# TIERS/multi-modal-loam

Hardware: AMD Instinct MI355X
Metric: scans/s (feature-extract+kNN+10 GN iters) on 16-ring x1800 + Livox 24k fused cloud (higher is better)
Workload: dtype f32/f64; 1 GPU; BASELINE configs[1]: fused VLP-16 16x1800 + Livox Horizon 24000 scan (52800 pts), local map 200000 pts, 1 association pass (thres_dist 25), 10 GN iterations, W=1; resident_slots=8192, stream_lanes=2, distinct_scans=64, map_tiles_touched=43, map_tiles_complete=43, parallelism=scan-sharded x1, device=AMD Radeon Graphics, cus=256

## Files before the change

multi-modal-loam_amd/csrc/knn5_dev.h:

```cpp

__device__ __forceinline__ int cell_coord(float v, float o, float inv, int dim) {
    int c = (int)floorf((v - o) * inv);
    return c < 0 ? 0 : (c >= dim ? dim - 1 : c);
}

struct Knn5 {
    unsigned long long key[5];
};
constexpr unsigned long long KNN_EMPTY = (0x7f800000ull << 32) | 0x7fffffffull;
__device__ __forceinline__ unsigned long long knn_key(float d, int id) {
    return ((unsigned long long)__float_as_uint(d) << 32) | (unsigned)id;
}
__device__ __forceinline__ float knn_d(const Knn5& k, int j) { return __uint_as_float((unsigned)(k.key[j] >> 32)); }
__device__ __forceinline__ int knn_id(const Knn5& k, int j) { return (int)(unsigned)k.key[j]; }
__device__ __forceinline__ void knn_init(Knn5& k) {
#pragma unroll
    for (int i = 0; i < 5; ++i) k.key[i] = KNN_EMPTY;
}
__device__ __forceinline__ unsigned long long sel64(bool c, unsigned long long a, unsigned long long b) {
    const unsigned lo = __builtin_unpredictable(c) ? (unsigned)a : (unsigned)b;
    const unsigned hi = __builtin_unpredictable(c) ? (unsigned)(a >> 32) : (unsigned)(b >> 32);
    return ((unsigned long long)hi << 32) | lo;
}
__device__ __forceinline__ void knn_insert_key(Knn5& k, unsigned long long x) {
    const bool lt0 = x < k.key[0], lt1 = x < k.key[1], lt2 = x < k.key[2], lt3 = x < k.key[3], lt4 = x < k.key[4];
    const unsigned long long c1 = sel64(lt0, k.key[0], x), c2 = sel64(lt1, k.key[1], x), c3 = sel64(lt2, k.key[2], x),
                             c4 = sel64(lt3, k.key[3], x);
    k.key[4] = sel64(lt4, c4, k.key[4]);
    k.key[3] = sel64(lt3, c3, k.key[3]);
    k.key[2] = sel64(lt2, c2, k.key[2]);
    k.key[1] = sel64(lt1, c1, k.key[1]);
    k.key[0] = sel64(lt0, x, k.key[0]);
}
__device__ __forceinline__ void knn_insert(Knn5& k, float dd, int ii) {
    const unsigned long long x = knn_key(dd, ii);
    if (!(x < k.key[4])) return;
    knn_insert_key(k, x);
}

__device__ __forceinline__ void scan_range(const float4* __restrict__ pts, const uint16_t* __restrict__ tags, int mytag,
                                           int s, int e, float qx, float qy, float qz, Knn5& k) {
    for (int i0 = s; i0 < e; i0 += 4) {
        float4 p[4];
        int tg[4];
#pragma unroll
        for (int u = 0; u < 4; ++u) {
            const unsigned i = (unsigned)min(i0 + u, e - 1);
            p[u] = pts[i];
            tg[u] = tags ? (int)tags[i] : mytag;
        }
#pragma unroll
        for (int u = 0; u < 4; ++u) {
            float dx = qx - p[u].x, dy = qy - p[u].y, dz = qz - p[u].z;
            float r = 0;
            r += dx * dx;
            r += dy * dy;
            r += dz * dz;
            const unsigned long long x = (i0 + u >= e || tg[u] != mytag) ? ~0ull : knn_key(r, (int)__float_as_uint(p[u].w));
            if (x < k.key[4]) knn_insert_key(k, x);
        }
    }
}

struct KnnQuery {
    float qx, qy, qz, inset;
    float fx, fy, fz;
    int hx, hy, hz;
};

__device__ __forceinline__ KnnQuery knn_query(const MmlGrid& g, float qx, float qy, float qz) {
    KnnQuery q;
    q.qx = qx;
    q.qy = qy;
    q.qz = qz;
    const float fx = (qx - g.origin[0]) * g.inv_cell, fy = (qy - g.origin[1]) * g.inv_cell,
                fz = (qz - g.origin[2]) * g.inv_cell;
    q.fx = fx;
    q.fy = fy;
    q.fz = fz;
    q.hx = (int)floorf(fx);
    q.hy = (int)floorf(fy);
    q.hz = (int)floorf(fz);
    float inset = fminf(fminf(fminf(fx - q.hx, q.hx + 1 - fx), fminf(fy - q.hy, q.hy + 1 - fy)),
                        fminf(fz - q.hz, q.hz + 1 - fz));
    q.inset = (inset > 0.f) ? inset : 0.f;
    return q;
}

__device__ __forceinline__ bool knn_done(const MmlGrid& g, float inset, int r, float d5, float max_d2) {
    float rho = ((float)r + inset) * g.cell;
    rho = rho - 1e-3f * g.cell;
    if (!(rho > 0.f)) return false;
    const float rho2 = rho * rho;
    return d5 < rho2 || rho2 >= max_d2;
}

__device__ __forceinline__ void scan_shell_row(const MmlGrid& g, const KnnQuery& q, int r, int y, int z, Knn5& k,
                                               int mytag = -1, float bound = INFINITY) {
    const int DX = g.dim[0], DY = g.dim[1], DZ = g.dim[2];
    if (y < 0 || y >= DY || z < 0 || z >= DZ) return;
    int xlo = -1, xhi = DX;
    if (bound < INFINITY) {
        const float gy = y > q.hy ? (float)y - q.fy : (y < q.hy ? q.fy - (float)(y + 1) : 0.f);
        const float gz = z > q.hz ? (float)z - q.fz : (z < q.hz ? q.fz - (float)(z + 1) : 0.f);
        const float reach = sqrtf(bound * 1.00001f) * g.inv_cell + 4e-3f;
        const float w2 = reach * reach - (gy * gy + gz * gz);
        if (w2 < 0.f) return;
        const float w = sqrtf(w2);
        xlo = (int)floorf(fmaxf(q.fx - w, -1.f));
        xhi = (int)floorf(fminf(q.fx + w, (float)DX));
    }
    const int x0 = q.hx - r, x1 = q.hx + r;
    const bool face = (z == q.hz - r || z == q.hz + r || y == q.hy - r || y == q.hy + r);
    const int rowbase = DX * (y + DY * z);
    if (face) {
        const int xa = max(max(x0, 0), xlo), xb = min(min(x1, DX - 1), xhi);
        if (xa <= xb)
            scan_range(g.pts, g.tags, mytag, g.cell_start[rowbase + xa], g.cell_start[rowbase + xb + 1], q.qx, q.qy, q.qz, k);
    } else {
        if (x0 >= 0 && x0 < DX && x0 >= xlo)
            scan_range(g.pts, g.tags, mytag, g.cell_start[rowbase + x0], g.cell_start[rowbase + x0 + 1], q.qx, q.qy, q.qz, k);
        if (x1 >= 0 && x1 < DX && x1 != x0 && x1 <= xhi)
            scan_range(g.pts, g.tags, mytag, g.cell_start[rowbase + x1], g.cell_start[rowbase + x1 + 1], q.qx, q.qy, q.qz, k);
    }
}

template <int STRIDE>
__device__ __forceinline__ void scan_shell_rows4(const MmlGrid& g, const KnnQuery& q, int r, int ylo, int wy, int zlo, int nrows,
                                                 int t, Knn5& k, int mytag, float bound) {
    const int DX = g.dim[0], DY = g.dim[1];
    const float reach = sqrtf(bound * 1.00001f) * g.inv_cell + 4e-3f;
    const float reach2 = reach * reach;
    const int x0 = q.hx - r, x1 = q.hx + r;
    unsigned ia[8], ib[8];
#pragma unroll
    for (int u = 0; u < 4; ++u) {
        const int tu = t + u * STRIDE;
        const int y = ylo + tu % wy, z = zlo + tu / wy;
        const float gy = y > q.hy ? (float)y - q.fy : (y < q.hy ? q.fy - (float)(y + 1) : 0.f);
        const float gz = z > q.hz ? (float)z - q.fz : (z < q.hz ? q.fz - (float)(z + 1) : 0.f);
        const float w2 = reach2 - (gy * gy + gz * gz);
        const bool in = tu < nrows && !(w2 < 0.f);
        const float w = sqrtf(fmaxf(w2, 0.f));
        const int xlo = (int)floorf(fmaxf(q.fx - w, -1.f)), xhi = (int)floorf(fminf(q.fx + w, (float)DX));
        const bool face = (z == q.hz - r || z == q.hz + r || y == q.hy - r || y == q.hy + r);
        const int rowbase = DX * (y + DY * z);
        const int xa = max(max(x0, 0), xlo), xb = min(min(x1, DX - 1), xhi);
        const bool va = in && (face ? xa <= xb : (x0 >= 0 && x0 < DX && x0 >= xlo));
        const bool vb = in && !face && x1 >= 0 && x1 < DX && x1 != x0 && x1 <= xhi;
        ia[2 * u] = va ? (unsigned)(rowbase + (face ? xa : x0)) : 0u;
        ib[2 * u] = va ? (unsigned)(rowbase + (face ? xb : x0) + 1) : 0u;
        ia[2 * u + 1] = vb ? (unsigned)(rowbase + x1) : 0u;
        ib[2 * u + 1] = vb ? (unsigned)(rowbase + x1 + 1) : 0u;
    }
    int s[8], e[8];
#pragma unroll
    for (int v = 0; v < 8; ++v) {
        s[v] = g.cell_start[ia[v]];
        e[v] = g.cell_start[ib[v]];
    }
    unsigned todo = 0;
#pragma unroll
    for (int v = 0; v < 8; ++v) todo |= (s[v] < e[v] ? 1u : 0u) << v;
#pragma unroll 1
    while (todo) {
        const int v = __ffs((int)todo) - 1;
        todo &= todo - 1;
        int ss = s[0], ee = e[0];
#pragma unroll
        for (int j = 1; j < 8; ++j) {
            ss = v == j ? s[j] : ss;
            ee = v == j ? e[j] : ee;
        }
        scan_range(g.pts, g.tags, mytag, ss, ee, q.qx, q.qy, q.qz, k);
    }
}

__device__ __constant__ const signed char kRing1Row[9][2] = {{0, 0}, {-1, 0}, {1, 0}, {0, -1}, {0, 1}, {-1, -1}, {1, -1}, {-1, 1}, {1, 1}};

__device__ __forceinline__ bool scan_rings01(const MmlGrid& g, const KnnQuery& q, int rmax, float max_d2, Knn5& k, int mytag) {
    scan_shell_row(g, q, 0, q.hy, q.hz, k, mytag);
    if (knn_done(g, q.inset, 0, knn_d(k, 4), max_d2)) return true;
    if (rmax < 1) return false;
#pragma unroll 1
    for (int t = 0; t < 9; ++t) scan_shell_row(g, q, 1, q.hy + kRing1Row[t][0], q.hz + kRing1Row[t][1], k, mytag, knn_d(k, 4));
    return knn_done(g, q.inset, 1, knn_d(k, 4), max_d2);
}

__device__ __forceinline__ unsigned long long knn_head(const Knn5& k, int head) {
    unsigned long long key = KNN_EMPTY;
#pragma unroll
    for (int s = 0; s < 5; ++s)
        if (head == s) key = k.key[s];
    return key;
}
__device__ __forceinline__ unsigned long long shfl_xor_u64(unsigned long long v, int o) {
    const unsigned lo = __shfl_xor((unsigned)v, o), hi = __shfl_xor((unsigned)(v >> 32), o);
    return ((unsigned long long)hi << 32) | lo;
}
template <int SPAN>
__device__ __forceinline__ void lanes_merge5(const Knn5& local, Knn5& out) {
    int head = 0;
#pragma unroll
    for (int r = 0; r < 5; ++r) {
        const unsigned long long mine = knn_head(local, head);
        unsigned long long m = mine;
#pragma unroll
        for (int o = SPAN / 2; o > 0; o >>= 1) {
            const unsigned long long other = shfl_xor_u64(m, o);
            m = other < m ? other : m;
        }
        out.key[r] = m;
        if (mine == m && (unsigned)(m >> 32) < 0x7f800000u) head++;
    }
}

__device__ void knn5_search(const MmlGrid& g, bool valid, float qx, float qy, float qz, float max_d2, Knn5& k) {
    knn_init(k);
    const KnnQuery q = knn_query(g, qx, qy, qz);
    const int rgrid = max(max(max(q.hx, g.dim[0] - 1 - q.hx), max(q.hy, g.dim[1] - 1 - q.hy)), max(q.hz, g.dim[2] - 1 - q.hz));
    const float rf = ceilf(sqrtf(max_d2) * g.inv_cell) + 1.f;
    const int rmax = rf < (float)rgrid ? (int)rf : max(rgrid, 0);
    bool pending = false;
    if (valid) {
        pending = !scan_rings01(g, q, rmax, max_d2, k, -1);
        if (rmax < 2) pending = false;
    }
    unsigned long long todo = __ballot(pending);
    const int lane = threadIdx.x & 63;
    while (todo) {
        const int src = __ffsll((long long)todo) - 1;
        todo &= todo - 1;
        KnnQuery s;
        s.qx = __shfl(q.qx, src);
        s.qy = __shfl(q.qy, src);
        s.qz = __shfl(q.qz, src);
        s.inset = __shfl(q.inset, src);
        s.fx = __shfl(q.fx, src);
        s.fy = __shfl(q.fy, src);
        s.fz = __shfl(q.fz, src);
        s.hx = __shfl(q.hx, src);
        s.hy = __shfl(q.hy, src);
        s.hz = __shfl(q.hz, src);
        Knn5 loc;
        if (lane == src)
            loc = k;
        else
            knn_init(loc);
        Knn5 best;
        knn_init(best);
        const int rmax_s = __shfl(rmax, src);
        const int rnear = max(max(max(-s.hx, s.hx - (g.dim[0] - 1)), max(-s.hy, s.hy - (g.dim[1] - 1))),
                              max(-s.hz, s.hz - (g.dim[2] - 1)));
        for (int r = max(2, rnear); r <= rmax_s; ++r) {
            const float bnd = fminf(knn_d(best, 4), __shfl(knn_d(k, 4), src));
            const int ylo = max(s.hy - r, 0), yhi = min(s.hy + r, g.dim[1] - 1), zlo = max(s.hz - r, 0), zhi = min(s.hz + r, g.dim[2] - 1);
            const int wy = yhi - ylo + 1, wz = zhi - zlo + 1;
            if (wy > 0 && wz > 0)
                for (int t = lane; t < wy * wz; t += 64)
                    scan_shell_row(g, s, r, ylo + (t % wy), zlo + (t / wy), loc, -1, fminf(bnd, knn_d(loc, 4)));
            lanes_merge5<64>(loc, best);
            if (knn_done(g, s.inset, r, knn_d(best, 4), max_d2)) break;
        }
        if (lane == src) k = best;
    }
}
```

multi-modal-loam_amd/csrc/map_assoc.hip:

```cpp
#include <math.h>
#include <stdlib.h>

#include <cstring>
#include <string.h>

#include "mml_internal.h"
#include "voxel_sort_dev.h"

namespace {

struct GridDev {
    float ox, oy, oz, inv_cell, cell;
    int dx, dy, dz, ncell;
};

#include "knn5_dev.h"

__global__ void k_cell_keys(const float4* pts, int m, GridDev g, unsigned* keys, unsigned* vals) {
    int i = blockIdx.x * blockDim.x + threadIdx.x;
    if (i >= m) return;
    float4 p = pts[i];
    int cx = cell_coord(p.x, g.ox, g.inv_cell, g.dx);
    int cy = cell_coord(p.y, g.oy, g.inv_cell, g.dy);
    int cz = cell_coord(p.z, g.oz, g.inv_cell, g.dz);
// ... 324 lines not shown
    float a11 = 0, a12 = 0, a13 = 0, a22 = 0, a23 = 0, a33 = 0;
#pragma unroll
    for (int j = 0; j < 5; j++) {
        float ax = nx[j] - cx, ay = ny[j] - cy, az = nz[j] - cz;
        a11 += ax * ax;
        a12 += ax * ay;
        a13 += ax * az;
        a22 += ay * ay;
        a23 += ay * az;
        a33 += az * az;
    }
    a11 /= 5;
    a12 /= 5;
    a13 /= 5;
    a22 /= 5;
    a23 /= 5;
    a33 /= 5;
    double ud[3];
    eig3_sym(a11, a12, a22, a13, a23, a33, m.ev, ud);
    m.cx = cx;
    m.cy = cy;
    m.cz = cz;
    if (!(m.ev[2] > 3 * m.ev[1])) return false;
    m.p1[0] = cx + 0.1 * ud[0];
    m.p1[1] = cy + 0.1 * ud[1];
    m.p1[2] = cz + 0.1 * ud[2];
    m.p2[0] = cx - 0.1 * ud[0];
    m.p2[1] = cy - 0.1 * ud[1];
    m.p2[2] = cz - 0.1 * ud[2];
    return true;
}

struct PlaneModel5 {
    double X[3];
    float pa, pb, pc, pd;
    double proj[3];
};
__device__ __forceinline__ bool plane_model5(const float* nx, const float* ny, const float* nz, float sx, float sy, float sz,
                                             PlaneModel5& m) {
    double A[5][3];
#pragma unroll
    for (int j = 0; j < 5; j++) {
        A[j][0] = nx[j];
        A[j][1] = ny[j];
        A[j][2] = nz[j];
    }
    plane_fit5(A, m.X);
    float pa = m.X[0], pb = m.X[1], pc = m.X[2], pd = 1;
    float ps = sqrtf(pa * pa + pb * pb + pc * pc);
    pa /= ps;
    pb /= ps;
    pc /= ps;
    pd /= ps;
    m.pa = pa;
    m.pb = pb;
    m.pc = pc;
    m.pd = pd;
    bool planeValid = true;
#pragma unroll
    for (int j = 0; j < 5; j++) {
        if (fabs((double)(pa * nx[j] + pb * ny[j] + pc * nz[j] + pd)) > 0.2) {
            planeValid = false;
            break;
        }
    }
    if (!planeValid) return false;
    double dist = pa * sx + pb * sy + pc * sz + pd;
    m.proj[0] = (double)sx - dist * (double)pa;
    m.proj[1] = (double)sy - dist * (double)pb;
    m.proj[2] = (double)sz - dist * (double)pc;
    return true;
}

__device__ __forceinline__ bool fit_and_store(const AssocParams& P, int kind, int b, int i, const float4 f, const double* T,
                                              float sx, float sy, float sz, bool ok, const Knn5& k, const float4* mp) {
    if (kind == 0) {
        MmlLineFactor out;
        out.src = -1;
        out.error = 0;
        if (ok) {
            float nx[5], ny[5], nz[5];
#pragma unroll
            for (int j = 0; j < 5; j++) {
                float4 q = mp[knn_id(k, j)];
                nx[j] = q.x;
                ny[j] = q.y;
                nz[j] = q.z;
            }
            LineModel5 m;
            if (line_model5(nx, ny, nz, m)) {
                const float x1 = m.p1[0], y1 = m.p1[1], z1 = m.p1[2], x2 = m.p2[0], y2 = m.p2[1], z2 = m.p2[2];
                out.ori[0] = f.x;
                out.ori[1] = f.y;
                out.ori[2] = f.z;
                out.p1[0] = x1;
                out.p1[1] = y1;
                out.p1[2] = z1;
                out.p2[0] = x2;
                out.p2[1] = y2;
                out.p2[2] = z2;
                out.src = i;
                double Px, Py, Pz;
                tf_point(T, f.x, f.y, f.z, Px, Py, Pz);
                double ax = x1, ay = y1, az = z1, bx = x2, by = y2, bz = z2;
                double l12 = sqrt((ax - bx) * (ax - bx) + (ay - by) * (ay - by) + (az - bz) * (az - bz));
                double c0 = (Px - ax) * (Py - by) - (Px - bx) * (Py - ay);
                double c1 = (Px - ax) * (Pz - bz) - (Px - bx) * (Pz - az);
                double c2 = (Py - ay) * (Pz - bz) - (Py - by) * (Pz - az);
                double a012 = sqrt(c0 * c0 + c1 * c1 + c2 * c2);
                out.error = a012 / l12;
            }
        }
        if (out.src >= 0) P.lf[(size_t)b * P.MF + i] = out;
        return out.src >= 0;
    } else {
        MmlPlaneFactor out;
        out.src = -1;
        out.error = 0;
        out._pad = 0;
        if (ok) {
            float nx[5], ny[5], nz[5];
#pragma unroll
            for (int j = 0; j < 5; j++) {
                float4 q = mp[knn_id(k, j)];
                nx[j] = q.x;
                ny[j] = q.y;
                nz[j] = q.z;
            }
            PlaneModel5 m;
            if (plane_model5(nx, ny, nz, sx, sy, sz, m)) {
                out.ori[0] = f.x;
                out.ori[1] = f.y;
                out.ori[2] = f.z;
                out.omega[0] = m.pa;
                out.omega[1] = m.pb;
                out.omega[2] = m.pc;
                out.proj[0] = m.proj[0];
                out.proj[1] = m.proj[1];
                out.proj[2] = m.proj[2];
                double Px, Py, Pz;
                tf_point(T, f.x, f.y, f.z, Px, Py, Pz);
                double ex = Px - out.proj[0], ey = Py - out.proj[1], ez = Pz - out.proj[2];
                out.error = sqrt((ex * ex + ey * ey) + ez * ez);
                out.src = i;
            }
        }
        if (out.src >= 0) P.pf[(size_t)b * P.MF + i] = out;
        return out.src >= 0;
    }
}

__global__ __launch_bounds__(128) void k_model_fit5(int op, const void* in_, long n, void* out_) {
    const long i = (long)blockIdx.x * 128 + threadIdx.x;
    if (i >= n) return;
    if (op == MML_FIT_EIG3) {
        const double* a = (const double*)in_ + 6 * i;
        double* o = (double*)out_ + 12 * i;
        double ev[3], v0[3], v1[3], v2[3];
        eig3_sym(a[0], a[1], a[2], a[3], a[4], a[5], ev, v2, v0, v1);
        for (int r = 0; r < 3; ++r) {
            o[r] = ev[r];
            o[3 + r] = v0[r];
            o[6 + r] = v1[r];
            o[9 + r] = v2[r];
        }
    } else if (op == MML_FIT_QR) {
        const double* a = (const double*)in_ + 15 * i;
        double* o = (double*)out_ + 4 * i;
        double A[5][3], X[3];
        int rank = 0;
        for (int r = 0; r < 5; ++r)
            for (int c = 0; c < 3; ++c) A[r][c] = a[3 * r + c];
        plane_fit5(A, X, &rank);
        o[0] = X[0];
        o[1] = X[1];
        o[2] = X[2];
        o[3] = rank;
    } else if (op == MML_FIT_LINE || op == MML_FIT_PLANE) {
        const int w = op == MML_FIT_LINE ? 15 : 18;
        const float* a = (const float*)in_ + w * i;
        float nx[5], ny[5], nz[5];
        for (int j = 0; j < 5; j++) {
            nx[j] = a[3 * j];
            ny[j] = a[3 * j + 1];
            nz[j] = a[3 * j + 2];
        }
        if (op == MML_FIT_LINE) {
            double* o = (double*)out_ + 13 * i;
            LineModel5 m;
            const bool ok = line_model5(nx, ny, nz, m);
            o[0] = ok ? 1 : 0;
            o[1] = m.cx;
            o[2] = m.cy;
            o[3] = m.cz;
            for (int r = 0; r < 3; ++r) {
                o[4 + r] = m.ev[r];
                o[7 + r] = ok ? m.p1[r] : 0.f;
                o[10 + r] = ok ? m.p2[r] : 0.f;
            }
        } else {
            double* o = (double*)out_ + 11 * i;
            PlaneModel5 m;
            const bool ok = plane_model5(nx, ny, nz, a[15], a[16], a[17], m);
            o[0] = ok ? 1 : 0;
            o[1] = m.X[0];
            o[2] = m.X[1];
            o[3] = m.X[2];
            o[4] = m.pa;
            o[5] = m.pb;
            o[6] = m.pc;
            o[7] = m.pd;
            for (int r = 0; r < 3; ++r) o[8 + r] = ok ? m.proj[r] : 0.0;
        }
    } else if (op == MML_FIT_OPS_F64) {
        const double* a = (const double*)in_ + 2 * i;
        double* o = (double*)out_ + 2 * i;
        o[0] = sqrt(a[0]);
        o[1] = a[0] / a[1];
    } else {
        const float* a = (const float*)in_ + 2 * i;
        float* o = (float*)out_ + 2 * i;
        o[0] = sqrtf(a[0]);
        o[1] = a[0] / a[1];
    }
}

constexpr int AP_THREADS = 256;
__global__ __launch_bounds__(AP_THREADS) void k_assoc_prefix(int first, int count, int B, const int* ft_n, int* work_off, int* hard_count) {
    __shared__ int s_wsum[16];
    const int tid = threadIdx.x, lane = tid & 63, wave = tid >> 6;
    if (tid == 0) *hard_count = 0;
    const int nitems = 2 * count;
    int acc = 0;
    for (int t0 = 0; t0 < nitems; t0 += 4 * AP_THREADS) {
        int v[4], x[4];
#pragma unroll
        for (int q = 0; q < 4; ++q) {
            const int it = t0 + q * AP_THREADS + tid;
            v[q] = 0;
            if (it < nitems) {
                const int kind = it / count, slot = it % count;
                const int nf = ft_n[kind * B + first + slot];
                v[q] = nf > 0 ? (nf + 127) / 128 : 0;
            }
        }
#pragma unroll
        for (int q = 0; q < 4; ++q) {
            int xx = v[q];
#pragma unroll
            for (int o = 1; o < 64; o <<= 1) {
                const int y = __shfl_up(xx, o);
                if (lane >= o) xx += y;
            }
            x[q] = xx;
            if (lane == 63) s_wsum[q * 4 + wave] = xx;
        }
        __syncthreads();
        int tile = 0, base[4] = {0, 0, 0, 0};
#pragma unroll
        for (int w = 0; w < 16; ++w) {
            const int t = s_wsum[w];
            tile += t;
#pragma unroll
            for (int q = 0; q < 4; ++q) base[q] += w < q * 4 + wave ? t : 0;
        }
#pragma unroll
        for (int q = 0; q < 4; ++q) {
            const int it = t0 + q * AP_THREADS + tid;
            if (it < nitems) work_off[it] = acc + base[q] + x[q] - v[q];
        }
        acc += tile;
        __syncthreads();
    }
    if (tid == 0) work_off[nitems] = acc;
}

constexpr int REC_NONE = 0, REC_READY = 1, REC_QUEUED = 2;
__device__ __forceinline__ int4* assoc_rec(const AssocParams& P, int kind, int b, int i) {
    return kind == 0 ? reinterpret_cast<int4*>(P.lf + (size_t)b * P.MF + i) : reinterpret_cast<int4*>(P.pf + (size_t)b * P.MF + i);
}
static_assert(sizeof(MmlLineFactor) >= 32 && sizeof(MmlLineFactor) % 16 == 0, "record parking needs 32 aligned bytes");
static_assert(sizeof(MmlPlaneFactor) >= 32 && sizeof(MmlPlaneFactor) % 16 == 0, "record parking needs 32 aligned bytes");

__device__ __forceinline__ int assoc_item(const AssocParams& P, int w) {
    int lo = 0, hi = 2 * P.count;
    while (hi - lo > 1) {
        const int mid = (lo + hi) >> 1;
        if (P.work_off[mid] <= w)
            lo = mid;
        else
            hi = mid;
    }
    return lo;
}

constexpr int HARD_REDO = 1 << 30;
constexpr int HARD_FRESH = 1 << 29;
#ifndef MML_AW_SEARCH
#define MML_AW_SEARCH 8
#define MML_AW_FIT 4
#define MML_AW_HARD 1
#endif
__global__ __launch_bounds__(128) __attribute__((amdgpu_waves_per_eu(MML_AW_SEARCH))) void k_associate(AssocParams P) {
    const int nitems = 2 * P.count;
    const int total = P.work_off[nitems];
    for (int w = blockIdx.x; w < total; w += gridDim.x) {
        const int item = assoc_item(P, w);
        const int kind = item / P.count, slot = item % P.count;
        const int b = slot + P.first;
        const int i = (w - P.work_off[item]) * 128 + threadIdx.x;
        const int nf = P.ft_n[kind * P.B + b];
        if (i >= nf) continue;
        int4* rec = assoc_rec(P, kind, b, i);
        const double* T = P.Twl + 16 * slot;
        const float4 f = P.ft[kind][(size_t)b * P.MF + i];
        double wx, wy, wz;
        tf_point(T, f.x, f.y, f.z, wx, wy, wz);
        const float sx = wx, sy = wy, sz = wz;
        const int cube = find_used_map(sx, sy, sz, P.cen);
        const int stage = (cube != 5000 && P.have_g[kind] && P.cube_cnt[kind][cube] > (kind == 0 ? 100 : 50)) ? 0 : 1;
        if (cube == 5000 || isnan(sx) || isnan(sy) || isnan(sz) || (stage == 1 && !(P.map_m[kind] > 20))) {
            rec[1] = make_int4(0, 0, REC_NONE, 0);
            continue;
        }
        if (P.fresh_all) {
            const int hw = atomicAdd(P.hard_count, 1);
            P.hard_list[hw] = make_int4(slot, kind, i, stage | (cube << 1) | HARD_FRESH);
            rec[1] = make_int4(0, 0, REC_QUEUED, 0);
            continue;
        }
        const int ukind = __builtin_amdgcn_readfirstlane(kind);
        Knn5 k;
        knn_init(k);
        bool done = false;
        int rmax = 0;
        if (stage == 0) {
            const MmlGrid& g = P.gg[ukind];
            const KnnQuery q = knn_query(g, sx, sy, sz);
            rmax = (int)ceilf(sqrtf(P.thres) * g.inv_cell) + 1;
            done = scan_rings01(g, q, rmax, P.thres, k, cube);
        } else {
            const MmlGrid& g = P.g[ukind];
            const KnnQuery q = knn_query(g, sx, sy, sz);
            rmax = (int)ceilf(sqrtf(P.thres) * g.inv_cell) + 1;
            done = scan_rings01(g, q, rmax, P.thres, k, -1);
        }
        if (!done && rmax >= 2) {
            const int hw = atomicAdd(P.hard_count, 1);
            P.hard_list[hw] = make_int4(slot, kind, i, stage | (cube << 1));
            float* hd = P.hard_knn + 10 * (size_t)hw;
#pragma unroll
            for (int j = 0; j < 5; ++j) {
                hd[j] = knn_d(k, j);
                hd[5 + j] = __int_as_float(knn_id(k, j));
            }
            rec[1] = make_int4(0, 0, REC_QUEUED, 0);
            continue;
        }
        rec[0] = make_int4(knn_id(k, 0), knn_id(k, 1), knn_id(k, 2), knn_id(k, 3));
        rec[1] = make_int4(knn_id(k, 4), __float_as_int(knn_d(k, 4)), REC_READY | (stage << 2), cube);
    }
}

__global__ __launch_bounds__(128) __attribute__((amdgpu_waves_per_eu(MML_AW_FIT))) void k_associate_fit_all(AssocParams P) {
    const int nitems = 2 * P.count;
    const int total = P.work_off[nitems];
    for (int w = blockIdx.x; w < total; w += gridDim.x) {
        const int item = assoc_item(P, w);
        const int kind = item / P.count, slot = item % P.count;
        const int b = slot + P.first;
        const int i = (w - P.work_off[item]) * 128 + threadIdx.x;
        const int nf = P.ft_n[kind * P.B + b];
        if (i >= nf) continue;
        const int4* rec = assoc_rec(P, kind, b, i);
        const int4 r0 = rec[0], r1 = rec[1];
        const int state = r1.z & 3, stage = r1.z >> 2, cube = r1.w;
        if (state == REC_QUEUED) continue;
        if (state == REC_NONE) {
            store_none(P, kind, b, i);
            continue;
        }
        const double* T = P.Twl + 16 * slot;
        const float4 f = P.ft[kind][(size_t)b * P.MF + i];
        double wx, wy, wz;
        tf_point(T, f.x, f.y, f.z, wx, wy, wz);
        const float sx = wx, sy = wy, sz = wz;
        Knn5 k;
        knn_init(k);
        const float d5 = __int_as_float(r1.y);
        k.key[0] = knn_key(d5, r0.x);
        k.key[1] = knn_key(d5, r0.y);
        k.key[2] = knn_key(d5, r0.z);
        k.key[3] = knn_key(d5, r0.w);
        k.key[4] = knn_key(d5, r1.x);
        const bool ok = (double)d5 < P.thres_d;
        const bool stored = fit_and_store(P, kind, b, i, f, T, sx, sy, sz, ok, k, stage == 0 ? P.gmap_orig[kind] : P.map_orig[kind]);
        if (!stored) {
            if (stage == 0 && P.map_m[kind] > 20) {
                const int hw = atomicAdd(P.hard_count, 1);
                P.hard_list[hw] = make_int4(slot, kind, i, (cube << 1) | HARD_REDO);
            } else {
                store_none(P, kind, b, i);
            }
        }
    }
}


template <int SPAN>
__global__ __launch_bounds__(256) __attribute__((amdgpu_waves_per_eu(MML_AW_HARD))) void k_associate_hard(AssocParams P, int round) {
    const int gl = threadIdx.x & (SPAN - 1);
    const int group = (blockIdx.x * 256 + threadIdx.x) / SPAN;
    const int ngroups = (gridDim.x * 256) / SPAN;
    const int total = *P.hard_count;
    for (int w0 = 0; w0 < total; w0 += ngroups) {
        const int w = w0 + group;
        bool live = w < total;
        int slot = 0, kind = 0, i = 0, b = P.first, stage = 1, cube = 0;
        bool fresh = false;
        float sx = 0, sy = 0, sz = 0;
        Knn5 loc, best;
        knn_init(loc);
        knn_init(best);
        if (live) {
            const int4 e = P.hard_list[w];
            if ((round == 1) != ((e.w & HARD_REDO) != 0)) live = false;
            slot = e.x;
            kind = e.y;
            i = e.z;
            stage = round == 1 ? 1 : (e.w & 1);
            cube = (e.w >> 1) & 0x3fff;
            fresh = (e.w & HARD_FRESH) != 0;
            b = slot + P.first;
        }
        if (live) {
            const float4 f = P.ft[kind][(size_t)b * P.MF + i];
            double wx, wy, wz;
            tf_point(P.Twl + 16 * slot, f.x, f.y, f.z, wx, wy, wz);
            sx = wx;
            sy = wy;
            sz = wz;
            if (round == 0 && gl == 0 && !fresh) {
                const float* hd = P.hard_knn + 10 * (size_t)w;
#pragma unroll
                for (int j = 0; j < 5; ++j) {
                    loc.key[j] = knn_key(hd[j], __float_as_int(hd[5 + j]));
                }
            }
        }
        const int r0 = (round == 0 && !fresh) ? 2 : 0;
        const float start_d5 = __shfl(knn_d(loc, 4), (threadIdx.x & 63) & ~(SPAN - 1));
        MmlGrid g = P.g[0];
        {
            const bool k1 = kind == 1, s0 = stage == 0;
            const MmlGrid &a = P.g[1], &c = P.gg[0], &d = P.gg[1];
#define MML_PICK(field) g.field = s0 ? (k1 ? d.field : c.field) : (k1 ? a.field : g.field)
            MML_PICK(pts);
            MML_PICK(cell_start);
            MML_PICK(tags);
            MML_PICK(origin[0]);
            MML_PICK(origin[1]);
            MML_PICK(origin[2]);
            MML_PICK(cell);
            MML_PICK(inv_cell);
            MML_PICK(dim[0]);
            MML_PICK(dim[1]);
            MML_PICK(dim[2]);
#undef MML_PICK
        }
        const int mytag = stage == 0 ? cube : -1;
        const KnnQuery q = knn_query(g, sx, sy, sz);
        const int rmax = live ? (int)ceilf(sqrtf(P.thres) * g.inv_cell) + 1 : 0;
        bool sdone = !live;
        const int rnear = max(max(max(-q.hx, q.hx - (g.dim[0] - 1)), max(-q.hy, q.hy - (g.dim[1] - 1))), max(-q.hz, q.hz - (g.dim[2] - 1)));
        const int rs = max(r0, rnear);
        if (!sdone && (r0 > rmax || (rs > r0 && (rs > rmax || knn_done(g, q.inset, rs - 1, start_d5, P.thres))))) {
            sdone = true;
            lanes_merge5<SPAN>(loc, best);
        }
        for (int r = rs;; ++r) {
            if (!sdone && r > rmax) sdone = true;
            if (__all(sdone)) break;
            if (!sdone) {
                const int ylo = max(q.hy - r, 0), yhi = min(q.hy + r, g.dim[1] - 1), zlo = max(q.hz - r, 0), zhi = min(q.hz + r, g.dim[2] - 1);
                const int wy = yhi - ylo + 1, wz = zhi - zlo + 1;
                if (wy > 0 && wz > 0)
                    for (int t = gl; t < wy * wz; t += 4 * SPAN) {
                        const float bound = fminf(fminf(fminf(knn_d(best, 4), knn_d(loc, 4)), start_d5), P.thres);
                        scan_shell_rows4<SPAN>(g, q, r, ylo, wy, zlo, wy * wz, t, loc, mytag, bound);
                    }
            }
            lanes_merge5<SPAN>(loc, best);
            if (!sdone && knn_done(g, q.inset, r, knn_d(best, 4), P.thres)) sdone = true;
        }
        if (live && gl == 0) {
            float* hd = P.hard_knn + 10 * (size_t)w;
#pragma unroll
            for (int j = 0; j < 5; ++j) {
                hd[j] = knn_d(best, j);
                hd[5 + j] = __int_as_float(knn_id(best, j));
            }
        }
    }
}

__global__ __launch_bounds__(128) void k_associate_fit(AssocParams P, int round) {
    const int total = *P.hard_count;
    for (int w = blockIdx.x * 128 + threadIdx.x; w < total; w += gridDim.x * 128) {
        const int4 e = P.hard_list[w];
        if ((round == 1) != ((e.w & HARD_REDO) != 0)) continue;
        const int slot = e.x, kind = e.y, i = e.z, b = slot + P.first;
        const int stage = round == 1 ? 1 : (e.w & 1);
        const float4 f = P.ft[kind][(size_t)b * P.MF + i];
        double wx, wy, wz;
        tf_point(P.Twl + 16 * slot, f.x, f.y, f.z, wx, wy, wz);
        const float sx = wx, sy = wy, sz = wz;
        Knn5 best;
        const float* hd = P.hard_knn + 10 * (size_t)w;
#pragma unroll
        for (int j = 0; j < 5; ++j) {
            best.key[j] = knn_key(hd[j], __float_as_int(hd[5 + j]));
        }
        const bool ok = (double)knn_d(best, 4) < P.thres_d;
        const bool stored = fit_and_store(P, kind, b, i, f, P.Twl + 16 * slot, sx, sy, sz, ok, best,
                                          stage == 0 ? P.gmap_orig[kind] : P.map_orig[kind]);
        if (!stored) {
            if (stage == 0 && P.map_m[kind] > 20)
                P.hard_list[w].w = e.w | HARD_REDO;
            else
                store_none(P, kind, b, i);
        }
        if (round == 1) P.hard_list[w].w = e.w & ~HARD_REDO;
    }
}

__global__ __launch_bounds__(256) void k_assoc_stats(int first, int B, int MF, const int* ft_n, const MmlLineFactor* lf,
                                                    const MmlPlaneFactor* pf, double* stats) {
    __shared__ double s_red[4][13];
    const int b = blockIdx.x + first;
    const int tid = threadIdx.x, lane = tid & 63, wave = tid >> 6;
    double acc[13];
    for (int k = 0; k < 13; ++k) acc[k] = 0;
    const int nl = ft_n[b], np = ft_n[B + b];
    for (int i = tid; i < nl; i += 256) {
        const MmlLineFactor& f = lf[(size_t)b * MF + i];
        if (f.src >= 0) {
            acc[0] += 1;
            if (fabs(f.error) > 1e-5) acc[2] += 1;
        }
    }
    for (int i = tid; i < np; i += 256) {
        const MmlPlaneFactor& f = pf[(size_t)b * MF + i];
        if (f.src >= 0) {
            acc[1] += 1;
            if (fabs(f.error) > 1e-5) acc[3] += 1;
            for (int r = 0; r < 3; ++r)
                for (int c = 0; c < 3; ++c) acc[4 + 3 * r + c] += (double)f.omega[r] * (double)f.omega[c];
        }
    }
    for (int k = 0; k < 13; ++k) {
        double v = acc[k];
        for (int o = 32; o > 0; o >>= 1) v += __shfl_xor(v, o);
        if (lane == 0) s_red[wave][k] = v;
    }
    __syncthreads();
    if (tid < 13) stats[16 * b + tid] = (s_red[0][tid] + s_red[1][tid]) + (s_red[2][tid] + s_red[3][tid]);
}

}

extern "C" int mml_model_fit5(mml_ctx* ctx, int op, const void* in, long n, void* out) {
    static const size_t in_bytes[6] = {6 * sizeof(double), 15 * sizeof(double), 15 * sizeof(float),
                                       18 * sizeof(float), 2 * sizeof(double),  2 * sizeof(float)};
    static const size_t out_bytes[6] = {12 * sizeof(double), 4 * sizeof(double), 13 * sizeof(double),
                                        11 * sizeof(double), 2 * sizeof(double), 2 * sizeof(float)};
    if (!ctx || !in || !out || n < 0 || op < 0 || op > MML_FIT_OPS_F32 || n > (long)1 << 26) return MML_ERR_INVALID;
    if (n == 0) return MML_OK;
    int rc = mml_sync_all(ctx);
    if (rc != MML_OK) return rc;
    MmlTemp<char> t_in, t_out;
    bool ok = t_in.alloc(in_bytes[op] * (size_t)n) == hipSuccess && t_out.alloc(out_bytes[op] * (size_t)n) == hipSuccess;
    void *d_in = t_in.d, *d_out = t_out.d;
    ok = ok && hipMemcpy(d_in, in, in_bytes[op] * (size_t)n, hipMemcpyHostToDevice) == hipSuccess;
    if (ok) {
        hipLaunchKernelGGL(k_model_fit5, dim3((unsigned)((n + 127) / 128)), dim3(128), 0, MML_STREAM(ctx), op, (const void*)d_in, n, d_out);
        ok = hipGetLastError() == hipSuccess && hipStreamSynchronize(MML_STREAM(ctx)) == hipSuccess;
    }
    ok = ok && hipMemcpy(out, d_out, out_bytes[op] * (size_t)n, hipMemcpyDeviceToHost) == hipSuccess;
    return ok ? MML_OK : MML_ERR_HIP;
}

static int build_grid_into(mml_ctx* ctx, MmlGrid& g, float4* orig, const float* h_xyz, int m, float cell,
                           const uint16_t* d_tag_orig) {
    hipStream_t s = MML_STREAM(ctx);
    g.m = m;
    if (m == 0) {
        g.dim[0] = g.dim[1] = g.dim[2] = 1;
        g.ncell = 1;
        g.cell = 1.f;
        g.inv_cell = 1.f;
        g.origin[0] = g.origin[1] = g.origin[2] = 0.f;
        MML_HIP(hipMemsetAsync(g.cell_start, 0, 2 * sizeof(int), s));
        return MML_OK;
    }
    if (h_xyz) {
        std::vector<float4> tmp((size_t)m);
        for (int i = 0; i < m; ++i) tmp[i] = make_float4(h_xyz[3 * i], h_xyz[3 * i + 1], h_xyz[3 * i + 2], 0.f);
        MML_HIP(hipMemcpyAsync(orig, tmp.data(), sizeof(float4) * (size_t)m, hipMemcpyHostToDevice, s));
        MML_HIP(hipStreamSynchronize(s));
    }
    MmlStageScope t(ctx, "map_build");
    const int init[6] = MML_BBOX_EMPTY;
    int* d_bbox = ctx->d_misc;
    MML_HIP(hipMemcpyAsync(d_bbox, init, sizeof(init), hipMemcpyHostToDevice, s));
    hipLaunchKernelGGL(k_bbox, dim3(256), dim3(256), 0, s, orig, m, d_bbox);
    int bbox_keys[6];
    MML_HIP(hipMemcpyAsync(bbox_keys, d_bbox, sizeof(bbox_keys), hipMemcpyDeviceToHost, s));
    MML_HIP(hipStreamSynchronize(s));
    float bbox[6];
    for (int c = 0; c < 6; ++c) bbox[c] = mml_funkey(bbox_keys[c]);
    const long long max_cells = (long long)4 * ctx->MM + 4096;
    const int blocks = (m + 255) / 256;
    int dim[3];
    for (int round = 0;; ++round) {
        for (;;) {
            long long total = 1;
            for (int c = 0; c < 3; ++c) {
                dim[c] = (int)floorf((bbox[3 + c] - bbox[c]) / cell) + 1;
                if (dim[c] < 1) dim[c] = 1;
                total *= dim[c];
            }
            if (total <= max_cells) break;
            cell *= 1.26f;
        }
        g.cell = cell;
        g.inv_cell = 1.0f / cell;
        for (int c = 0; c < 3; ++c) {
            g.origin[c] = bbox[c];
            g.dim[c] = dim[c];
        }
        g.ncell = dim[0] * dim[1] * dim[2];
        GridDev gd{g.origin[0], g.origin[1], g.origin[2], g.inv_cell, g.cell, dim[0], dim[1], dim[2], g.ncell};
        hipLaunchKernelGGL(k_cell_keys, dim3(blocks), dim3(256), 0, s, orig, m, gd, ctx->map_keys, ctx->map_vals);
        int bits = 1;
        while ((1ll << bits) < g.ncell) ++bits;
        const int rt = mml_sort_pairs(ctx, ctx->sort_tmp, ctx->map_keys, ctx->map_keys2, ctx->map_vals, ctx->map_vals2, (size_t)m, bits, s);
        if (rt != MML_OK) return rt;
        int* d_occ = ctx->d_misc + 16;
// ... 194 lines not shown
```

Measured before the change: 449,800 scans/s.

## Flatten ring-1 kNN scan into one pruned piece list streamed from LDS

Ring-1 neighbourhood scanning now gathers all cell ranges at once, trimming the x-extent of each row against the current 5th-best distance. The non-empty ranges go into a per-thread piece table in shared memory, and the points are then streamed in one loop, unrolled by four, instead of nine separate row scans. The goal is less per-row loop overhead and divergence, more loads in flight, and fewer points scanned. In exchange it adds about 10 KB of LDS per block, which may lower occupancy, and it keeps a fallback path for very long ranges.

```diff
diff --git a/multi-modal-loam_amd/csrc/knn5_dev.h b/multi-modal-loam_amd/csrc/knn5_dev.h
--- a/multi-modal-loam_amd/csrc/knn5_dev.h
+++ b/multi-modal-loam_amd/csrc/knn5_dev.h
@@ -184,6 +184,103 @@
     if (rmax < 1) return false;
 #pragma unroll 1
     for (int t = 0; t < 9; ++t) scan_shell_row(g, q, 1, q.hy + kRing1Row[t][0], q.hz + kRing1Row[t][1], k, mytag, knn_d(k, 4));
+    return knn_done(g, q.inset, 1, knn_d(k, 4), max_d2);
+}
+
+constexpr int KNN_FLAT_PIECES = 10;
+#ifndef MML_KNN_FLAT_MAXLEN
+#define MML_KNN_FLAT_MAXLEN 0xffff
+#endif
+static_assert(MML_KNN_FLAT_MAXLEN >= 1 && MML_KNN_FLAT_MAXLEN <= 0xffff, "piece lengths are stored in 16 bits");
+template <int NT>
+struct KnnFlatTable {
+    unsigned start[KNN_FLAT_PIECES * NT];
+    unsigned short len[KNN_FLAT_PIECES * NT];
+};
+static_assert(sizeof(KnnFlatTable<128>) <= 10 * 1024 && sizeof(KnnFlatTable<128>) / 128 <= 80, "piece table exceeds its LDS budget");
+
+template <int NT>
+__device__ __forceinline__ bool scan_rings01_flat(const MmlGrid& g, const KnnQuery& q, int rmax, float max_d2, Knn5& k, int mytag,
+                                                  KnnFlatTable<NT>& tab, int tid) {
+    scan_shell_row(g, q, 0, q.hy, q.hz, k, mytag);
+    if (knn_done(g, q.inset, 0, knn_d(k, 4), max_d2)) return true;
+    if (rmax < 1) return false;
+    const int DX = g.dim[0], DY = g.dim[1], DZ = g.dim[2];
+    const float bound = knn_d(k, 4);
+    const float reach = sqrtf(bound * 1.00001f) * g.inv_cell + 4e-3f;
+    const float reach2 = reach * reach;
+    const int x0 = q.hx - 1, x1 = q.hx + 1;
+    int s[KNN_FLAT_PIECES], e[KNN_FLAT_PIECES];
+#pragma unroll
+    for (int t = 0; t < 9; ++t) {
+        const int y = q.hy + kRing1Row[t][0], z = q.hz + kRing1Row[t][1];
+        const float gy = y > q.hy ? (float)y - q.fy : (y < q.hy ? q.fy - (float)(y + 1) : 0.f);
+        const float gz = z > q.hz ? (float)z - q.fz : (z < q.hz ? q.fz - (float)(z + 1) : 0.f);
+        const float w2 = reach2 - (gy * gy + gz * gz);
+        const bool in = y >= 0 && y < DY && z >= 0 && z < DZ && !(w2 < 0.f);
+        const float w = sqrtf(fmaxf(w2, 0.f));
+        const int xlo = (int)floorf(fmaxf(q.fx - w, -1.f)), xhi = (int)floorf(fminf(q.fx + w, (float)DX));
+        const int rowbase = DX * (y + DY * z);
+        if (t == 0) {
+            const bool va = in && x0 >= 0 && x0 < DX && x0 >= xlo;
+            const bool vb = in && x1 >= 0 && x1 < DX && x1 <= xhi;
+            s[0] = g.cell_start[va ? (unsigned)(rowbase + x0) : 0u];
+            e[0] = g.cell_start[va ? (unsigned)(rowbase + x0 + 1) : 0u];
+            s[1] = g.cell_start[vb ? (unsigned)(rowbase + x1) : 0u];
+            e[1] = g.cell_start[vb ? (unsigned)(rowbase + x1 + 1) : 0u];
+        } else {
+            const int xa = max(max(x0, 0), xlo), xb = min(min(x1, DX - 1), xhi);
+            const bool va = in && xa <= xb;
+            s[t + 1] = g.cell_start[va ? (unsigned)(rowbase + xa) : 0u];
+            e[t + 1] = g.cell_start[va ? (unsigned)(rowbase + xb + 1) : 0u];
+        }
+    }
+    int np = 0, total = 0;
+    bool big = false;
+#pragma unroll
+    for (int v = 0; v < KNN_FLAT_PIECES; ++v) {
+        const int len = e[v] - s[v];
+        if (len > 0) {
+            tab.start[np * NT + tid] = (unsigned)s[v];
+            tab.len[np * NT + tid] = (unsigned short)len;
+            ++np;
+            total += len;
+            big |= len > MML_KNN_FLAT_MAXLEN;
+        }
+    }
+    if (big) {
+#pragma unroll 1
+        for (int t = 0; t < 9; ++t) scan_shell_row(g, q, 1, q.hy + kRing1Row[t][0], q.hz + kRing1Row[t][1], k, mytag, knn_d(k, 4));
+        return knn_done(g, q.inset, 1, knn_d(k, 4), max_d2);
+    }
+    int pi = 0, pend = 0;
+    unsigned cur = 0;
+#pragma unroll 1
+    for (int n = 0; n < total; n += 4) {
+        float4 p[4];
+        int tg[4];
+#pragma unroll
+        for (int u = 0; u < 4; ++u) {
+            if (n + u == pend && n + u < total) {
+                cur = tab.start[pi * NT + tid];
+                pend += (int)tab.len[pi * NT + tid];
+                ++pi;
+            }
+            const unsigned i = n + u < total ? cur++ : cur - 1u;
+            p[u] = g.pts[i];
+            tg[u] = g.tags ? (int)g.tags[i] : mytag;
+        }
+#pragma unroll
+        for (int u = 0; u < 4; ++u) {
+            float dx = q.qx - p[u].x, dy = q.qy - p[u].y, dz = q.qz - p[u].z;
+            float r = 0;
+            r += dx * dx;
+            r += dy * dy;
+            r += dz * dz;
+            const unsigned long long x = (n + u >= total || tg[u] != mytag) ? ~0ull : knn_key(r, (int)__float_as_uint(p[u].w));
+            if (x < k.key[4]) knn_insert_key(k, x);
+        }
+    }
     return knn_done(g, q.inset, 1, knn_d(k, 4), max_d2);
 }
 
diff --git a/multi-modal-loam_amd/csrc/map_assoc.hip b/multi-modal-loam_amd/csrc/map_assoc.hip
--- a/multi-modal-loam_amd/csrc/map_assoc.hip
+++ b/multi-modal-loam_amd/csrc/map_assoc.hip
@@ -650,6 +650,7 @@
 #define MML_AW_HARD 1
 #endif
 __global__ __launch_bounds__(128) __attribute__((amdgpu_waves_per_eu(MML_AW_SEARCH))) void k_associate(AssocParams P) {
+    __shared__ KnnFlatTable<128> s_pieces;
     const int nitems = 2 * P.count;
     const int total = P.work_off[nitems];
     for (int w = blockIdx.x; w < total; w += gridDim.x) {
@@ -686,12 +687,12 @@
             const MmlGrid& g = P.gg[ukind];
             const KnnQuery q = knn_query(g, sx, sy, sz);
             rmax = (int)ceilf(sqrtf(P.thres) * g.inv_cell) + 1;
-            done = scan_rings01(g, q, rmax, P.thres, k, cube);
+            done = scan_rings01_flat(g, q, rmax, P.thres, k, cube, s_pieces, (int)threadIdx.x);
         } else {
             const MmlGrid& g = P.g[ukind];
             const KnnQuery q = knn_query(g, sx, sy, sz);
             rmax = (int)ceilf(sqrtf(P.thres) * g.inv_cell) + 1;
-            done = scan_rings01(g, q, rmax, P.thres, k, -1);
+            done = scan_rings01_flat(g, q, rmax, P.thres, k, -1, s_pieces, (int)threadIdx.x);
         }
         if (!done && rmax >= 2) {
             const int hw = atomicAdd(P.hard_count, 1);
```

Measured after the change: 450,700 scans/s, median of 2. Within noise of the previous version (+0.2%).
